# fan-ziqi/robot_lab

Hardware: AMD Instinct MI355X
Metric: env-steps/sec (whole node) at 4096 envs/GPU, A1 Velocity-Rough (higher is better)
Workload: dtype f32; 1 GPU; RobotLab-Isaac-Velocity-Rough-Unitree-A1-v0, 4096 envs/GPU, random actions U(-1,1), seed 42+rank; envs_per_gpu=4096, parallelism=env-shard x1, step_kernel=specialised (spec_id 1), envs_per_wavefront=4

## Files before the change

### robot_lab_amd/csrc/env_step.h

```cpp
#pragma once
#include <type_traits>

#include "env_spec.h"
#include "env_tables.h"

#if defined(RL_PHASE_MARKS) && defined(__HIP_DEVICE_COMPILE__)
#define RL_PHASE(id, name) asm volatile("; PHASE " name)
#elif defined(RL_PHASE_CLOCK) && defined(__HIP_DEVICE_COMPILE__)
#define RL_PHASE(id, name) this->phase_stamp(id)
#define RL_PHASE_START() (this->ph_t0 = 0, this->ph_cur = 0)
#define RL_PHASE_CLOCK_ON 1
#else
#define RL_PHASE(id, name) ((void)0)
#endif
#ifndef RL_PHASE_START
#define RL_PHASE_START() ((void)0)
#endif
constexpr int RL_PHASE_ROW0 = 24;
constexpr int RL_PHASE_SLOTS = 32;

namespace rl {

template <int N>
struct SymIdx {
  static constexpr int size = N * (N + 1) / 2;
  static constexpr int at(int i, int j) { return i <= j ? i * N - i * (i - 1) / 2 + (j - i) : j * N - j * (j - 1) / 2 + (i - j); }
};

template <int I, int N, class F>
RL_FN void static_for(F&& f) {
  if constexpr (I < N) {
    f(std::integral_constant<int, I>{});
    static_for<I + 1, N>(f);
  }
}
template <int I, class F>
RL_FN void static_for_down(F&& f) {
  if constexpr (I >= 0) {
    f(std::integral_constant<int, I>{});
    static_for_down<I - 1>(f);
  }
}

RL_FN float comp(V3 v, int i) { return i == 0 ? v.x : i == 1 ? v.y : v.z; }
RL_FN V3 unit(int i) { return {i == 0 ? 1.f : 0.f, i == 1 ? 1.f : 0.f, i == 2 ? 1.f : 0.f}; }
RL_FN V3 ld3(const float* p) { return {p[0], p[1], p[2]}; }

struct Uni {
  float dt, inv_dt, gravity, contact_k, contact_c, inv_phi_ref, contact_ct, contact_vdep, contact_vstick, limit_k, limit_c, force_threshold;
  float inv_hscale, x0, y0;
  int is_plane, nx, ny;
  double x0d, y0d, inv_hd;
  uint32_t trunk_restart;
};
template <class Ctx>
RL_FN Uni make_uni(const Ctx& ctx, const TaskTab& T) {
  Uni u;
  u.dt = ctx.uniform(T.dt); u.inv_dt = ctx.uniform(1.0f / T.dt); u.gravity = ctx.uniform(T.gravity);
  u.contact_k = ctx.uniform(T.contact_k); u.contact_c = ctx.uniform(T.contact_c); u.inv_phi_ref = ctx.uniform(1.0f / T.contact_phi_ref);
  u.contact_ct = ctx.uniform(T.contact_ct); u.contact_vdep = ctx.uniform(T.contact_vdep); u.contact_vstick = ctx.uniform(T.contact_vstick);
  u.limit_k = ctx.uniform(T.limit_k); u.limit_c = ctx.uniform(T.limit_c); u.force_threshold = ctx.uniform(T.force_threshold);
  u.inv_hscale = ctx.uniform(T.is_plane ? 1.0f : 1.0f / T.hscale); u.x0 = ctx.uniform(T.x0); u.y0 = ctx.uniform(T.y0);
  u.is_plane = ctx.uniform_i(T.is_plane); u.nx = ctx.uniform_i(T.nx); u.ny = ctx.uniform_i(T.ny);
  auto uni_d = [&](double v) {
    union { double d; int i[2]; } w;
    w.d = v;
    w.i[0] = ctx.uniform_i(w.i[0]); w.i[1] = ctx.uniform_i(w.i[1]);
    return w.d;
  };
// ... 490 lines not shown
    static_for<0, 3>([&](auto dc) __attribute__((always_inline)) {
      constexpr int D = 1 << decltype(dc)::value;
      float w[12] = {Rl.r0.x, Rl.r0.y, Rl.r0.z, Rl.r1.x, Rl.r1.y, Rl.r1.z, Rl.r2.x, Rl.r2.y, Rl.r2.z, pl.x, pl.y, pl.z};
      ctx.template sub_shr<D>(w);
      const M3 Rq{{w[0], w[1], w[2]}, {w[3], w[4], w[5]}, {w[6], w[7], w[8]}};
      const V3 pq{w[9], w[10], w[11]};
      const bool take = sub >= D;
      const M3 Rn = mul(Rq, Rl);
      const V3 pn = pq + mul(Rq, pl);
      Rl = select_m3(take, Rn, Rl);
      pl = select3(take, pn, pl);
    });
    const M3 Rj = mul(Ra, Rl);
    const V3 pj = pa + mul(Ra, pl);
    const V3 axj = mul(Rj, al_s);
    if (has) C.set(js, Rj, pj, axj);
    if constexpr (VEL) {
      const SV Sj{axj, cross(pj, axj)};
      const SV vj = Sj * (has ? qds : 0.f);
      float vs[6] = {vj.a.x, vj.a.y, vj.a.z, vj.l.x, vj.l.y, vj.l.z};
      static_for<0, 3>([&](auto dc) __attribute__((always_inline)) {
        constexpr int D = 1 << decltype(dc)::value;
        float w[6] = {vs[0], vs[1], vs[2], vs[3], vs[4], vs[5]};
        ctx.template sub_shr<D>(w);
        const bool take = sub >= D;
#pragma unroll
        for (int i = 0; i < 6; ++i) vs[i] += take ? w[i] : 0.f;
      });
      const SV Vj = Va + SV{{vs[0], vs[1], vs[2]}, {vs[3], vs[4], vs[5]}};
      const SV cj = crm(Vj, vj);
      float cs[6] = {cj.a.x, cj.a.y, cj.a.z, cj.l.x, cj.l.y, cj.l.z};
      static_for<0, 3>([&](auto dc) __attribute__((always_inline)) {
        constexpr int D = 1 << decltype(dc)::value;
        float w[6] = {cs[0], cs[1], cs[2], cs[3], cs[4], cs[5]};
        ctx.template sub_shr<D>(w);
        const bool take = sub >= D;
#pragma unroll
        for (int i = 0; i < 6; ++i) cs[i] += take ? w[i] : 0.f;
      });
      const SV aj = aa + SV{{cs[0], cs[1], cs[2]}, {cs[3], cs[4], cs[5]}};
      if (has) {
        float* w = va_words(js);
        st4(w, F4{Vj.a.x, Vj.a.y, Vj.a.z, Vj.l.x});
        st4(w + 4, F4{Vj.l.y, Vj.l.z, aj.a.x, aj.a.y});
        st4(w + 8, F4{aj.a.z, aj.l.x, aj.l.y, aj.l.z});
      }
    }
  }

  Ctx& ctx;
  const KState& S;
  const TablesT<TP>& T;
  const LaneTabT<TP>& L;
  const Uni u;
  int e, k, sub, li, Np;
  static constexpr int MAXOWN = SUB == 1 ? NBS : LaneTabT<TP>::template maxown<SUB>();
  int own[MAXOWN];
  static constexpr bool STATE_BUF = SUB == 1;
  float* lt;
  float* et;
  typename Ctx::StateBuf lt_b, et_b;
  uint32_t lt_off, et_off;
  struct BufRef {
    const typename Ctx::StateBuf& b;
    uint32_t voff, soff;
    RL_FN operator float() const { return Ctx::buf_ld(b, voff, soff); }
    RL_FN float operator=(float v) const { Ctx::buf_st(b, voff, soff, v); return v; }
  };
  struct PtrRef {
    float* p;
    RL_FN operator float() const { return *p; }
    RL_FN float operator=(float v) const { *p = v; return v; }
  };
  V3 pos, vlin, vang;
  Q4 quat;
  float q[JX], qd[JX], kp[JX], kd[JX], act[JX], prev_act[JX];
  V3 base_com;
  V3 wr_com;
  V3 extF, extT;
  float fric0[3];
  float tau_app[JX], qacc[JX];
  static constexpr int NOWN = LsFor<TP, Ctx::SUB>::NOWN;
  static constexpr bool GRAN = LsFor<TP, Ctx::SUB>::GRAN;
  LsMat<LSS, NOWN, 4, GRAN> tim;
  LsMat<LSS, NOWN, 3, GRAN> hist_n;
  LsMat<LSS, NOWN, 3, GRAN> cf;
  LsMat<LSS, NOWN, 3, GRAN> fric;

  RL_FN EnvLane(Ctx& c, const KState& s)
      : ctx(c), S(s), T(c.template tables<TablesT<TP>>()), L(c.template tables<TablesT<TP>>().lane[c.k()]), u(make_uni(c, c.template tables<TablesT<TP>>())), tim{c.template lane_scratch<GRAN>() + LS::TIM * LSS, {}}, hist_n{c.template lane_scratch<GRAN>() + LS::HIST * LSS, {}},
        cf{c.template lane_scratch<GRAN>() + LS::CF * LSS, {}}, fric{c.template lane_scratch<GRAN>() + LS::FRIC * LSS, {}} {
    e = ctx.env();
    k = ctx.k();
    sub = ctx.sub();
    li = k * SUB + sub;
    Np = S.Npad;
#pragma unroll
    for (int i = 0; i < MAXOWN; ++i) {
      if constexpr (SUB == 8) own[i] = -1;
      else own[i] = SUB == 1 ? i : (SUB == 2 ? L.own_slot2[sub & 1][i < LaneTabT<TP>::MAXOWN2 ? i : 0] : L.own_slot[sub & 3][i < LaneTabT<TP>::MAXOWN ? i : 0]);
    }
    if constexpr (SUB == 8) {
      int n = 0;
#pragma unroll
      for (int sl = 0; sl < NBS; ++sl) {
        const bool mine = (L.slot_body[sl] >= 0 || (sl == 0 && L.base_body_local >= 0)) && (L.slot_grp[sl] & 7) == sub;
#pragma unroll
        for (int i = 0; i < MAXOWN; ++i) own[i] = (mine && n == i) ? sl : own[i];
        n += mine ? 1 : 0;
      }
    }
    tim.set_own(own); hist_n.set_own(own); cf.set_own(own); fric.set_own(own);
    if constexpr (STATE_BUF) {
      lt_b = Ctx::state_buf(ctx.uniform_ptr(S.lane_state + (size_t)ctx.tile() * ((size_t)LY.NF_LANE * ROW)), (uint32_t)LY.NF_LANE * ROW * (uint32_t)sizeof(float));
      et_b = Ctx::state_buf(ctx.uniform_ptr(S.env_state + (size_t)ctx.tile() * ((size_t)LY.NF_ENV * EPT)), (uint32_t)LY.NF_ENV * (uint32_t)EPT * (uint32_t)sizeof(float));
      lt_off = (uint32_t)sizeof(float) * (uint32_t)(ctx.env_in_tile() * NLANE + k);
      et_off = (uint32_t)sizeof(float) * (uint32_t)ctx.env_in_tile();
    } else {
      lt = S.lane_state + (size_t)ctx.tile() * ((size_t)LY.NF_LANE * ROW) + (uint32_t)(ctx.env_in_tile() * NLANE + k);
      et = S.env_state + (size_t)ctx.tile() * ((size_t)LY.NF_ENV * EPT) + (uint32_t)ctx.env_in_tile();
    }
  }
#ifdef RL_PHASE_CLOCK_ON
  long long ph_t0 = 0;
  int ph_cur = 0;
  __device__ __forceinline__ void phase_stamp(int id) {
    __builtin_amdgcn_s_waitcnt(0);
    const long long t = (long long)__builtin_readcyclecounter();
    if (ctx.lane == 0 && ph_t0 != 0) {
      float* row = S.rew_terms + (size_t)RL_PHASE_ROW0 * (size_t)S.Npad + (size_t)ctx.tile() * RL_PHASE_SLOTS;
      row[ph_cur] += (float)(t - ph_t0);
    }
    ph_cur = id;
    __builtin_amdgcn_s_waitcnt(0);
    ph_t0 = (long long)__builtin_readcyclecounter();
  }
#endif
  RL_FN auto LF(int f) const {
    if constexpr (STATE_BUF) {
      const uint32_t o = (uint32_t)f * ROW * (uint32_t)sizeof(float);
      return __builtin_constant_p(f) ? BufRef{lt_b, lt_off, o} : BufRef{lt_b, lt_off + o, 0u};
    } else return PtrRef{lt + (uint32_t)f * ROW};
  }
  RL_FN auto EF(int f) const {
    if constexpr (STATE_BUF) {
      const uint32_t o = (uint32_t)f * (uint32_t)EPT * (uint32_t)sizeof(float);
      return __builtin_constant_p(f) ? BufRef{et_b, et_off, o} : BufRef{et_b, et_off + o, 0u};
    } else return PtrRef{et + (uint32_t)f * (uint32_t)EPT};
  }
  static constexpr bool M0 = TP::M0 != 0;
  static constexpr int G0 = M0 ? 1 : 0;
  RL_FN int grp_of(int it) const { return G0 + sub + SUB * it; }
  static constexpr bool slot_live(int it, int s) {
    const int lo = G0 + SUB * it, hi = lo + SUB - 1 < CL ? lo + SUB - 1 : CL;
    return spec_slot_any<SP>(s, SPL, lo, hi);
  }
  RL_FN bool owns_group(int g) const { return SUB == 1 || (g < G0 ? sub == 0 : ((g - G0) % SUB) == sub); }
  RL_FN bool on_base(int g, int s) const { return M0 && ((L.sph_base_mask >> (g * SPL + s)) & 1u) != 0u; }
  RL_FN static SV pick_sv(bool c, const SV& a, const SV& b) {
    return SV{{c ? a.a.x : b.a.x, c ? a.a.y : b.a.y, c ? a.a.z : b.a.z}, {c ? a.l.x : b.l.x, c ? a.l.y : b.l.y, c ? a.l.z : b.l.z}};
  }
  RL_FN uint32_t base_bits() const { return M0 ? L.sph_base_mask : ((1u << SPL) - 1u); }
  RL_FN bool owns_slot(int s) const { return owns_group(L.slot_grp[s]); }

  RL_FN void load() {
    pos = {EF(LY.EF_ROOT + 0), EF(LY.EF_ROOT + 1), EF(LY.EF_ROOT + 2)};
    quat = {EF(LY.EF_ROOT + 3), EF(LY.EF_ROOT + 4), EF(LY.EF_ROOT + 5), EF(LY.EF_ROOT + 6)};
    vlin = {EF(LY.EF_ROOT + 7), EF(LY.EF_ROOT + 8), EF(LY.EF_ROOT + 9)};
    vang = {EF(LY.EF_ROOT + 10), EF(LY.EF_ROOT + 11), EF(LY.EF_ROOT + 12)};
    extF = {EF(LY.EF_WRENCH + 0), EF(LY.EF_WRENCH + 1), EF(LY.EF_WRENCH + 2)};
    extT = {EF(LY.EF_WRENCH + 3), EF(LY.EF_WRENCH + 4), EF(LY.EF_WRENCH + 5)};
    base_com = {EF(LY.EF_BASE_COM + 0), EF(LY.EF_BASE_COM + 1), EF(LY.EF_BASE_COM + 2)};
    if (NW > 0) wr_com = {EF(LY.EF_WR_COM + 0), EF(LY.EF_WR_COM + 1), EF(LY.EF_WR_COM + 2)};
    else wr_com = base_com;
#pragma unroll
    for (int j = 0; j < CL; ++j) {
      q[j] = LF(LY.LF_Q + j);
      qd[j] = LF(LY.LF_QD + j);
      kp[j] = LF(LY.LF_KP + j);
      kd[j] = LF(LY.LF_KD + j);
      act[j] = LF(LY.LF_ACT + j);
    }
#pragma unroll
    for (int i = 0; i < NW; ++i) {
      q[CL + i] = EF(LY.EF_TQ + i);
      qd[CL + i] = EF(LY.EF_TQD + i);
      kp[CL + i] = EF(LY.EF_TKP + i);
      kd[CL + i] = EF(LY.EF_TKD + i);
      act[CL + i] = EF(LY.EF_TACT + i);
    }
#pragma unroll
    for (int j = 0; j < JX; ++j) {
      tau_app[j] = 0.f;
      qacc[j] = 0.f;
    }
    if (M0) {
#pragma unroll
      for (int t = 0; t < 3; ++t) fric0[t] = LF(LY.LF_FRICTION + t);
    }
#pragma unroll
    for (int i = 0; i < MAXOWN; ++i) {
      const int s = own[i];
      if (s < 0) continue;
      tim.st(s, F4{LF(LY.LF_TIMERS + s * 4 + 0), LF(LY.LF_TIMERS + s * 4 + 1), LF(LY.LF_TIMERS + s * 4 + 2), LF(LY.LF_TIMERS + s * 4 + 3)});
      fric.st(s, F4{LF(LY.LF_FRICTION + s * 3 + 0), LF(LY.LF_FRICTION + s * 3 + 1), LF(LY.LF_FRICTION + s * 3 + 2), 0.f});
      cf.st(s, F4{0.f, 0.f, 0.f, 0.f});
      hist_n.st(s, F4{0.f, 0.f, 0.f, 0.f});
    }
  }

  RL_FN void store() {
    if (li == 0) {
      EF(LY.EF_ROOT + 0) = pos.x; EF(LY.EF_ROOT + 1) = pos.y; EF(LY.EF_ROOT + 2) = pos.z;
      EF(LY.EF_ROOT + 3) = quat.w; EF(LY.EF_ROOT + 4) = quat.x; EF(LY.EF_ROOT + 5) = quat.y; EF(LY.EF_ROOT + 6) = quat.z;
      EF(LY.EF_ROOT + 7) = vlin.x; EF(LY.EF_ROOT + 8) = vlin.y; EF(LY.EF_ROOT + 9) = vlin.z;
      EF(LY.EF_ROOT + 10) = vang.x; EF(LY.EF_ROOT + 11) = vang.y; EF(LY.EF_ROOT + 12) = vang.z;
      EF(LY.EF_WRENCH + 0) = extF.x; EF(LY.EF_WRENCH + 1) = extF.y; EF(LY.EF_WRENCH + 2) = extF.z;
      EF(LY.EF_WRENCH + 3) = extT.x; EF(LY.EF_WRENCH + 4) = extT.y; EF(LY.EF_WRENCH + 5) = extT.z;
#pragma unroll
      for (int i = 0; i < NW; ++i) {
        EF(LY.EF_TQ + i) = q[CL + i];
        EF(LY.EF_TQD + i) = qd[CL + i];
        EF(LY.EF_TKP + i) = kp[CL + i];
        EF(LY.EF_TKD + i) = kd[CL + i];
        EF(LY.EF_TACT + i) = act[CL + i];
      }
    }
    if (sub == 0) {
#pragma unroll
      for (int j = 0; j < CL; ++j) {
        LF(LY.LF_Q + j) = q[j];
        LF(LY.LF_QD + j) = qd[j];
        LF(LY.LF_KP + j) = kp[j];
        LF(LY.LF_KD + j) = kd[j];
        LF(LY.LF_ACT + j) = act[j];
      }
    }
#pragma unroll
    for (int i = 0; i < MAXOWN; ++i) {
      const int s = own[i];
      if (s < 0 || (s == 0 && SUB > 1 && L.slot_body[0] < 0)) continue;
      const F4 t4 = tim.ld(s);
      LF(LY.LF_TIMERS + s * 4 + 0) = t4.x; LF(LY.LF_TIMERS + s * 4 + 1) = t4.y; LF(LY.LF_TIMERS + s * 4 + 2) = t4.z; LF(LY.LF_TIMERS + s * 4 + 3) = t4.w;
// ... 1170 lines not shown
```

### robot_lab_amd/csrc/env_terms.h

```cpp
#pragma once
#include "env_spec.h"
#include "env_step.h"

namespace rl {

enum RewKind {
  REW_TRACK_LIN_VEL_XY_EXP = 0, REW_TRACK_ANG_VEL_Z_EXP, REW_LIN_VEL_Z_L2, REW_ANG_VEL_XY_L2, REW_JOINT_TORQUES_L2,
  REW_JOINT_ACC_L2, REW_JOINT_POS_LIMITS, REW_JOINT_POWER, REW_STAND_STILL, REW_JOINT_POS_PENALTY, REW_JOINT_MIRROR,
  REW_ACTION_RATE_L2, REW_UNDESIRED_CONTACTS, REW_CONTACT_FORCES, REW_FEET_CONTACT_WITHOUT_CMD, REW_FEET_HEIGHT_BODY,
  REW_UPWARD, REW_FEET_AIR_TIME, REW_FEET_AIR_TIME_VARIANCE, REW_FEET_SLIDE, REW_FEET_GAIT, REW_FLAT_ORIENTATION_L2,
  REW_IS_TERMINATED, REW_JOINT_DEVIATION_L1, REW_JOINT_VEL_L2, REW_FEET_CONTACT, REW_FEET_STUMBLE, REW_FEET_HEIGHT,
  REW_TRACK_LIN_VEL_XY_YAW_FRAME_EXP, REW_TRACK_ANG_VEL_Z_WORLD_EXP, REW_FEET_AIR_TIME_POSITIVE_BIPED,
  REW_HANDSTAND_FEET_HEIGHT_EXP, REW_HANDSTAND_FEET_ON_AIR, REW_HANDSTAND_FEET_AIR_TIME, REW_HANDSTAND_ORIENTATION_L2, REW_BASE_HEIGHT_L2, REW_WHEEL_VEL_PENALTY,
  REW_FEET_DISTANCE_Y_EXP, REW_FEET_DISTANCE_XY_EXP, REW_ACTION_MIRROR, REW_ACTION_SYNC
};
enum ObsKind {
  OBS_BASE_LIN_VEL = 0, OBS_BASE_ANG_VEL, OBS_PROJECTED_GRAVITY, OBS_VELOCITY_COMMANDS, OBS_JOINT_POS_REL,
  OBS_JOINT_VEL_REL, OBS_LAST_ACTION, OBS_HEIGHT_SCAN, OBS_JOINT_POS_REL_NO_WHEEL
};

enum { JS_TAU2 = 0, JS_ACC2, JS_QD2, JS_LIMIT, JS_POWER, JS_DEV1, JS_DEV2, JS_DA2, JS_Q, JS_ABSQD, JS_ROWS };
enum { BT_HMAX = 0, BT_CA, BT_CC, BT_LA, BT_LC, BT_FX, BT_FY, BT_FZ, BT_PX, BT_PY, BT_PZ, BT_VX, BT_VY, BT_VZ, BT_NF };
static_assert(JS_ROWS == REW_JS_ROWS && BT_NF == REW_BT_NF && BT_FX == REW_BT_NS, "reward tables: LDS sizing in env_tables.h");

// ... 264 lines not shown
      }
      switch (R.kind) {
        case REW_UNDESIRED_CONTACTS: f = a0 * gate; break;
        case REW_CONTACT_FORCES: f = a0; break;
        case REW_FEET_CONTACT_WITHOUT_CMD: f = a0 * (cmd_norm < 0.1f ? 1.f : 0.f) * gate; break;
        case REW_FEET_CONTACT: f = (a0 != R.p[0] ? 1.f : 0.f) * moving * gate; break;
        case REW_FEET_AIR_TIME: f = a0 * moving * gate; break;
        case REW_HANDSTAND_FEET_AIR_TIME: f = a0; break;
        case REW_FEET_STUMBLE: f = (a0 > 0.f ? 1.f : 0.f) * gate; break;
        case REW_FEET_HEIGHT_BODY: case REW_FEET_HEIGHT: f = a0 * moving * gate; break;
        case REW_FEET_SLIDE: f = a0 * gate; break;
        case REW_FEET_AIR_TIME_POSITIVE_BIPED: f = (a0 == 1.f ? fminf(mn, R.p[0]) : 0.f) * moving * gate; break;
        case REW_HANDSTAND_FEET_HEIGHT_EXP: f = fexp(-a0 * frcp(R.p[0])); break;
        case REW_HANDSTAND_FEET_ON_AIR: f = a0 == 0.f ? 1.f : 0.f; break;
        case REW_FEET_AIR_TIME_VARIANCE: {
          const float inv_n = frcp(a0), inv_den = frcp(fmaxf(a0 - 1.f, 1.f));
          f = ((a2 - a1 * a1 * inv_n) + (a4 - a3 * a3 * inv_n)) * inv_den * gate;
        } break;
        default: break;
      }
    } break;
  }
  return f;
}


template <class Ctx, class TP, class SP = NoSpec>
struct EnvProgram : EnvLane<Ctx, TP, SP> {
  using Base = EnvLane<Ctx, TP, SP>;
  using ChainTP = typename Base::ChainTP;
  static constexpr Layout LY = Base::LY;
  static constexpr int CL = TP::CL, NW = TP::NW, JX = TP::JX, NBS = TP::NBS;
  using Base::ctx; using Base::S; using Base::T; using Base::L; using Base::e; using Base::k; using Base::sub; using Base::li; using Base::Np;
  static constexpr int SUB = Base::SUB;
  static constexpr int LPE = Base::LPE;
  using Base::pos; using Base::quat; using Base::vlin; using Base::vang; using Base::q; using Base::qd; using Base::kp; using Base::kd;
  using Base::act; using Base::prev_act; using Base::tim; using Base::cf; using Base::hist_n; using Base::tau_app; using Base::qacc;
  using Base::extF; using Base::extT; using Base::base_com; using Base::wr_com;

  V3 cmd;
  float heading_target, cmd_time_left, metric_xy, metric_yaw, push_left;
  static constexpr bool DEFER_LOG = SUB > 1;
  static constexpr int NACC_M = (MAX_T + LPE - 1) / LPE;
  float log_sum[NACC_M], log_mxy, log_myaw;
  bool is_heading, is_standing;
  int level, ttype;
  V3 origin;
  long long ep_len;
  M3 Rwb;
  V3 lin_b, ang_b, grav_b, lin_w;
  float yaw_c, yaw_s;

  RL_FN EnvProgram(Ctx& c, const KState& s) : Base(c, s) {}

  RL_FN void load_task() {
    cmd = {this->EF(LY.EF_CMD + CMD_VX), this->EF(LY.EF_CMD + CMD_VY), this->EF(LY.EF_CMD + CMD_WZ)};
    heading_target = this->EF(LY.EF_CMD + CMD_HEADING);
    cmd_time_left = this->EF(LY.EF_CMD + CMD_TIME_LEFT);
    metric_xy = this->EF(LY.EF_CMD + CMD_METRIC_XY);
    metric_yaw = this->EF(LY.EF_CMD + CMD_METRIC_YAW);
    push_left = this->EF(LY.EF_CMD + CMD_PUSH_LEFT);
    int f = S.flags[e];
    is_heading = f & 1;
    is_standing = (f >> 1) & 1;
    level = S.level[e];
    ttype = S.ttype[e];
    origin = {this->EF(LY.EF_ORIGIN + 0), this->EF(LY.EF_ORIGIN + 1), this->EF(LY.EF_ORIGIN + 2)};
    ep_len = S.ep_len[e];
  }
  RL_FN void store_task() {
    if (li != 0) return;
    this->EF(LY.EF_CMD + CMD_VX) = cmd.x; this->EF(LY.EF_CMD + CMD_VY) = cmd.y; this->EF(LY.EF_CMD + CMD_WZ) = cmd.z;
    this->EF(LY.EF_CMD + CMD_HEADING) = heading_target; this->EF(LY.EF_CMD + CMD_TIME_LEFT) = cmd_time_left;
    this->EF(LY.EF_CMD + CMD_METRIC_XY) = metric_xy; this->EF(LY.EF_CMD + CMD_METRIC_YAW) = metric_yaw; this->EF(LY.EF_CMD + CMD_PUSH_LEFT) = push_left;
    S.flags[e] = (is_heading ? 1 : 0) | (is_standing ? 2 : 0);
    S.level[e] = level;
    this->EF(LY.EF_ORIGIN + 0) = origin.x; this->EF(LY.EF_ORIGIN + 1) = origin.y; this->EF(LY.EF_ORIGIN + 2) = origin.z;
    S.ep_len[e] = ep_len;
    S.command_out[e * 3 + 0] = cmd.x; S.command_out[e * 3 + 1] = cmd.y; S.command_out[e * 3 + 2] = cmd.z;
  }

  RL_FN void derive() {
    Rwb = quat_to_mat(quat);
    V3 com_w = mul(Rwb, base_com);
    lin_w = vlin + cross(vang, com_w);
    lin_b = mulT(Rwb, lin_w);
    ang_b = mulT(Rwb, vang);
    grav_b = mulT(Rwb, V3{0.f, 0.f, -1.f});
    const float hn = frsqrt(fmaxf(Rwb.r0.x * Rwb.r0.x + Rwb.r1.x * Rwb.r1.x, 1e-30f));
    yaw_c = Rwb.r0.x * hn;
    yaw_s = Rwb.r1.x * hn;
  }

  RL_FN uint64_t uniform_u64(uint64_t v) const {
    return ((uint64_t)(uint32_t)ctx.uniform_i((int)(uint32_t)(v >> 32)) << 32) | (uint64_t)(uint32_t)ctx.uniform_i((int)(uint32_t)v);
  }
  RL_FN float U(uint32_t stream, uint32_t idx, float lo, float hi) const {
    return uniform_range(S.seed, (uint32_t)e, S.step_counter, stream, idx, lo, hi);
  }

  RL_FN void apply_command_draws(const float (&uw)[6]) {
    float rx0 = T.cmd_range[0][0], rx1 = T.cmd_range[0][1], ry0 = T.cmd_range[1][0], ry1 = T.cmd_range[1][1], rz0 = T.cmd_range[2][0], rz1 = T.cmd_range[2][1];
    float rh0 = T.cmd_range[3][0], rh1 = T.cmd_range[3][1], rel_h = T.cmd_rel_heading, rel_s = T.cmd_rel_standing, small = T.cmd_small_threshold;
    int use_heading = T.cmd_heading;
    rl_pin(rx0); rl_pin(rx1); rl_pin(ry0); rl_pin(ry1); rl_pin(rz0); rl_pin(rz1); rl_pin(rh0); rl_pin(rh1); rl_pin(rel_h); rl_pin(rel_s); rl_pin(small); rl_pin(use_heading);
    if (T.cur_lin != 0 || T.cur_ang != 0) {
// ... 841 lines not shown
        F[FEAT_JOINT + 2 * D + jid] = act[j];
        F[FEAT_JOINT + 3 * D + jid] = ((wheel >> (jid & 31)) & 1u) ? 0.f : qr;
      }
    }
    ctx.group_sync();
    const bool d0 = direct_group(T, 0), d1 = direct_group(T, 1);
    if (SUB == 1 && d0) write_group<true>(T.obs[0], F, S.obs_policy + (size_t)e * (size_t)T.policy_dim, 0u, cy, sy, scan_p, sp);
    else write_group<false>(T.obs[0], F, ctx.obs_stage(0), 0u, cy, sy, scan_p, sp);
    RL_PHASE(21, "obs.policy_done");
    if (SUB == 1 && d1) write_group<true>(T.obs[1], F, S.obs_critic + (size_t)e * (size_t)T.critic_dim, 1024u, cy, sy, scan_p, sp);
    else write_group<false>(T.obs[1], F, ctx.obs_stage(1), 1024u, cy, sy, scan_p, sp);
    RL_PHASE(22, "obs.flush");
    if (!(SUB == 1 && d0)) ctx.flush_obs(S.obs_policy, T.policy_dim, 0);
    if (!(SUB == 1 && d1)) ctx.flush_obs(S.obs_critic, T.critic_dim, 1);
  }

  RL_FN float* log_slot() const {
    return S.log + ((size_t)(S.step_counter & (uint32_t)(LOG_RING - 1)) * LOG_PARTS + (size_t)(ctx.tile() & (LOG_PARTS - 1))) * LOG_SIZE;
  }

  RL_FN void collect_cmd_levels(bool done) {
    if (!(T.cur_lin || T.cur_ang) || !done || e >= S.N || S.step_counter % (uint32_t)T.max_episode_length != 0u) return;
    for (int t = li; t < T.n_rewards; t += LPE) {
      const float v = S.ep_sums[(size_t)t * Np + e];
      if (T.cur_lin && t == T.cur_lin_term) { ctx.atomic_add(S.cmd_levels + CL_SUM_LIN, v); ctx.atomic_add(S.cmd_levels + CL_CNT_LIN, 1.f); }
      if (T.cur_ang && t == T.cur_ang_term) { ctx.atomic_add(S.cmd_levels + CL_SUM_ANG, v); ctx.atomic_add(S.cmd_levels + CL_CNT_ANG, 1.f); }
    }
  }
  RL_FN void write_dbg_views(float live) {
    if (S.dbg_torque == nullptr) return;
    if (sub == 0)
#pragma unroll
      for (int j = 0; j < JX; ++j) {
        if (TP::PAD && !L.joint_own[j]) continue;
        S.dbg_torque[(size_t)e * T.D + L.joint_id[j]] = live * tau_app[j];
        S.dbg_acc[(size_t)e * T.D + L.joint_id[j]] = live * qacc[j];
      }
#pragma unroll
    for (int s = 0; s < NBS; ++s) {
      int b = L.slot_body[s];
      if (b >= 0 && (s != 0 || L.owns_base_body) && this->owns_slot(s)) {
        float* o = S.dbg_cforce + ((size_t)e * T.n_bodies + b) * 3;
        const F4 fs = cf.ld(s);
        o[0] = live * fs.x; o[1] = live * fs.y; o[2] = live * fs.z;
      }
    }
  }
  RL_FN bool out_of_bounds() const {
    if (!T.term_oob || T.is_plane) return false;
    const float mw = (float)T.num_rows * T.tile_size + 2.f * T.border, mh = (float)T.num_cols * T.tile_size + 2.f * T.border;
    return fabsf(pos.x) > 0.5f * mw - T.oob_buffer || fabsf(pos.y) > 0.5f * mh - T.oob_buffer;
  }

  RL_FN void step() { step_front<false>(); }
  RL_FN void step_head() { step_front<true>(); }
  RL_FN void step_tail() {
    this->load();
    load_task();
    derive();
    const bool terminated = S.terminated[e] != 0, time_out = S.time_out[e] != 0;
    const bool t_oob = out_of_bounds();
    const bool t_timeout = T.term_time_out && ep_len >= (long long)T.max_episode_length;
    step_back<true>(terminated, time_out, t_timeout, t_oob, terminated);
  }

  template <bool HEAD>
  RL_FN void step_front() {
    constexpr size_t LOG_SLOT_WORDS = (size_t)LOG_PARTS * LOG_SIZE;
    const int log_tl = ctx.tile(), log_wl = ctx.env_in_tile() * LPE + li;
    float* log_pv = S.log + (size_t)((S.step_counter - 1u) & (uint32_t)(LOG_RING - 1)) * LOG_SLOT_WORDS;
    const float* log_pp = S.log + (size_t)((S.step_counter - 2u) & (uint32_t)(LOG_RING - 1)) * LOG_SLOT_WORDS;
    float log_fresh = 0.f, log_word = 0.f;
    if (log_tl < LOG_PARTS) {
      for (int p = 0; p < LOG_PARTS; ++p) log_fresh += log_pv[p * LOG_SIZE + LOG_FRESH];
      log_word = log_pp[log_tl * LOG_SIZE + log_wl];
    }
    float a_in[JX];
    {
      const float* arow = S.action_in + (size_t)(e < S.N ? e : 0) * T.D;
#pragma unroll
      for (int j = 0; j < JX; ++j) {
        const int jid = L.joint_id[j];
        a_in[j] = arow[TP::PAD && jid < 0 ? 0 : jid];
      }
    }
    RL_PHASE_START();
    RL_PHASE(0, "load");
    this->load();
    load_task();
    rl_pin(a_in);
    if (log_tl < LOG_PARTS) {
      float* nx = S.log + (size_t)((S.step_counter + 1u) & (uint32_t)(LOG_RING - 1)) * LOG_SLOT_WORDS;
      const bool inherit = log_fresh == 0.f;
      if (inherit && log_wl != LOG_FRESH) log_pv[log_tl * LOG_SIZE + log_wl] = log_word;
      nx[log_tl * LOG_SIZE + log_wl] = 0.f;
      for (int p = log_tl + S.Npad / (64 / LPE); p < LOG_PARTS; p += S.Npad / (64 / LPE)) {
        if (inherit && log_wl != LOG_FRESH) log_pv[p * LOG_SIZE + log_wl] = log_pp[p * LOG_SIZE + log_wl];
        nx[p * LOG_SIZE + log_wl] = 0.f;
      }
    }
    RL_PHASE(1, "action");
    float q_tgt[JX], qd_tgt[JX];
#pragma unroll
    for (int j = 0; j < JX; ++j) {
      prev_act[j] = act[j];
      const float a = (e < S.N && (!TP::PAD || L.joint_id[j] >= 0)) ? a_in[j] : 0.f;
      act[j] = a;
      float pr = clampf(a * L.a_scale[j] + L.a_off[j], L.a_lo[j], L.a_hi[j]);
      q_tgt[j] = L.action_is_vel[j] ? 0.f : pr;
      qd_tgt[j] = L.action_is_vel[j] ? pr : 0.f;
    }
#ifdef RL_ABL_SUBSTEPS
    if constexpr (Base::ABA) {
      this->substeps_aba(q_tgt, qd_tgt, RL_ABL_SUBSTEPS);
    } else
#endif
    if constexpr (Base::ABA) {
      this->substeps_aba(q_tgt, qd_tgt, T.decimation);
    } else {
      this->self_load();
      for (int s = 0; s < T.decimation; ++s) this->substep_aba_trunk(q_tgt, qd_tgt);
    }
    RL_PHASE(15, "terminations");
    ep_len += 1;
    derive();
    if constexpr (NW > 0) {
      ChainTP Cf = this->new_chain();
      this->kinematics(Cf);
      ctx.group_sync();
    }

    bool t_timeout = T.term_time_out && ep_len >= (long long)T.max_episode_length;
    const bool t_oob = out_of_bounds();
    bool t_illegal = false;
    if (T.term_illegal) {
      const uint64_t ill_mask = T.illegal_body_mask;
      const float ill_thr = T.illegal_threshold;
      float c = 0.f;
#pragma unroll
      for (int i = 0; i < Base::MAXOWN; ++i) {
        const int so = this->own[i], s = so < 0 ? 0 : so;
        const float h = hist_max(s);
// ... 137 lines not shown
```

### robot_lab_amd/csrc/rl_env_kernels.h

```cpp
#pragma once
#include <hip/hip_runtime.h>

#include <algorithm>
#include <cmath>
#include <cstdlib>
#include <mutex>
#include <string>

#define RL_FN __host__ __device__ __forceinline__
#include "env_aos.h"
#include "env_terms.h"

namespace {

using namespace rl;

template <int CTRL>
__device__ inline float dpp(float v) {
  return __int_as_float(__builtin_amdgcn_update_dpp(0, __float_as_int(v), CTRL, 0xF, 0xF, false));
}
template <int CTRL>
__device__ inline float dpp_move(float v) {
  return __int_as_float(__builtin_amdgcn_update_dpp(0, __float_as_int(v), CTRL, 0xF, 0xF, true));
}
// ... 173 lines not shown
  }
};

struct LdsPlan {
  int s0w, s1w;
  int fdim, rtdim, rsdim;
  int lb0, lbrec0, envs, tail;
  int rstage, stage0, stage1, fstage;
  int words;
};
template <class TP, int SUB>
RL_FN LdsPlan lds_plan(int policy_dim, int critic_dim, bool direct0, bool direct1, int D, int n_bodies, uint64_t rew_ext_mask, int n_rewards) {
  constexpr int EPT = 64 / (NLANE * SUB), LIMBS = 64 / SUB;
  using LS = typename LsFor<TP, SUB>::type;
  constexpr int STASH_WORDS = LsFor<TP, SUB>::STASH * LsFor<TP, SUB>::type::SSW * 64;
  constexpr int LB_FREE = TP::NW > 0 ? LbLayout<TP>::RECW * LIMBS : 0;
  LdsPlan P;
  P.s0w = (SUB == 1 && direct0) ? 0 : (EPT * policy_dim + 3) & ~3;
  P.s1w = (SUB == 1 && direct1) ? 0 : (EPT * critic_dim + 3) & ~3;
  P.fdim = feat_count(D);
  P.rtdim = rew_tab_words(D, n_bodies, rew_ext_mask);
  P.rsdim = rew_stage_words(n_rewards);
  int region = P.s0w + P.s1w + EPT * P.fdim;
  if (region < EPT * P.rtdim) P.s1w += EPT * P.rtdim - region, region = EPT * P.rtdim;
  if (SUB > 1 && region < EPT * RESET_RAND_WORDS) P.s1w += EPT * RESET_RAND_WORDS - region, region = EPT * RESET_RAND_WORDS;
  P.lb0 = LS::WORDS * 64;
  P.lbrec0 = P.lb0 + LbLayout<TP>::CHAINW * LIMBS;
  P.envs = P.lb0 + LbLayout<TP>::WORDS * LIMBS;
  P.tail = P.envs + EPT * LbLayout<TP>::ENV_WORDS;
  const bool alias = TP::NW == 0 && STASH_WORDS > 0 && EPT * P.rsdim + region <= STASH_WORDS;
  const bool alias_lb = TP::NW > 0 && EPT * P.rsdim + region <= LB_FREE;
  P.rstage = alias ? LS::CT * 64 : (alias_lb ? P.lbrec0 : P.tail);
  P.stage0 = P.rstage + EPT * P.rsdim;
  P.stage1 = P.stage0 + P.s0w;
  P.fstage = P.stage1 + P.s1w;
  P.words = (alias || alias_lb) ? P.tail : P.tail + EPT * P.rsdim + region;
  P.words = (P.words + 3) & ~3;
  return P;
}

extern __shared__ float4 smem4[];

#ifndef RL_LB
#define RL_LB(w) 256
#endif
template <class TP, int RESET, int SUB, int WGW, class SP = NoSpec>
__global__ __launch_bounds__(RL_LB(WGW)) void env_kernel(KState S, const void* __restrict__ Tgv, uint32_t wave_words) {
  using Ctx = WaveCtx<SUB>;
  using Tables = TablesT<TP>;
  const Tables* __restrict__ Tg = static_cast<const Tables*>(Tgv);
  float* smem = reinterpret_cast<float*>(smem4);
  Tables* Tl = reinterpret_cast<Tables*>(smem);
  const int lane = threadIdx.x & 63, wv = threadIdx.x >> 6;
  S.step_counter += *S.step_base;
  {
    const float4* src = reinterpret_cast<const float4*>(Tg);
    float4* dst = reinterpret_cast<float4*>(Tl);
    constexpr int TPB = 64 * WGW;
    constexpr int NIT = ((int)(sizeof(Tables) / 16) + TPB - 1) / TPB;
    const int n4 = (int)(S.table_bytes >> 4);
    float4 tmp[NIT];
#pragma unroll
    for (int it = 0; it < NIT; ++it) {
      const int i = (int)threadIdx.x + TPB * it;
      tmp[it] = src[i < n4 ? i : n4 - 1];
    }
#pragma unroll
    for (int it = 0; it < NIT; ++it) {
      const int i = (int)threadIdx.x + TPB * it;
      if (i < n4) dst[i] = tmp[it];
    }
  }
  if (WGW > 1) __syncthreads();
  else Ctx::wave_sync();
  const int TAB_F = (int)(S.table_bytes >> 2);
  const LdsPlan P = lds_plan<TP, SUB>(Tl->policy_dim, Tl->critic_dim, direct_group(*Tl, 0), direct_group(*Tl, 1), Tl->D, Tl->n_bodies, Tl->rew_ext_mask, Tl->n_rewards);
  Ctx ctx;
  ctx.T = Tl;
  ctx.Tg = Tgv;
  ctx.dim[0] = Tl->policy_dim;
  ctx.dim[1] = Tl->critic_dim;
  ctx.lscratch = smem + TAB_F + (WGW > 1 ? wv * wave_words : 0u);
  ctx.wtile = (int)blockIdx.x * WGW + wv;
  if (WGW > 1 && ctx.wtile >= S.Npad / Ctx::EPT) return;
  ctx.lbchain = ctx.lscratch + P.lb0 + (lane / SUB) * LbLayout<TP>::CHAINW;
  ctx.lbrec = ctx.lscratch + P.lbrec0 + (lane / SUB) * LbLayout<TP>::RECW;
  ctx.lbrec_stride = LbLayout<TP>::RECW;
  ctx.envs = ctx.lscratch + P.envs + (lane / Ctx::LPE) * LbLayout<TP>::ENV_WORDS;
  ctx.fdim = P.fdim;
  ctx.rtdim = P.rtdim;
  ctx.rsdim = P.rsdim;
  ctx.rstage = ctx.lscratch + P.rstage;
  ctx.stage[0] = ctx.lscratch + P.stage0;
  ctx.stage[1] = ctx.lscratch + P.stage1;
  ctx.fstage = ctx.lscratch + P.fstage;
  ctx.lane = lane;
  EnvProgram<Ctx, TP, SP> prog(ctx, S);
  if (RESET == 1)
    prog.reset_entry();
  else if (RESET == 2)
    prog.step_head();
  else
    prog.step();
}


struct LaunchCfg {
  int device = 0, n_cu = 256;
  int wg_waves = 4;
  bool wg_force = false;
};

template <class TP, int SUB, int WGW, class SP = NoSpec>
hipError_t launch_w(const LaunchCfg& cfg, const KState& S, const void* T, size_t lds1, hipStream_t st) {
  const int tiles = S.Npad / (16 / SUB);
  dim3 grid((tiles + WGW - 1) / WGW), block(64 * WGW);
  const uint32_t wave_words = (uint32_t)((lds1 - S.table_bytes) >> 2);
  const size_t lds = S.table_bytes + (size_t)WGW * (lds1 - S.table_bytes);
  constexpr bool HEAD = SUB == 4 && WGW == 1 && !SP::ON, RESET = WGW == 1 && !SP::ON;
  if (lds > 64 * 1024) {
    static size_t configured[64] = {};
    static std::mutex mu;
    std::lock_guard<std::mutex> lock(mu);
    size_t& have = configured[cfg.device & 63];
    if (lds > have) {
      hipError_t e = hipFuncSetAttribute(reinterpret_cast<const void*>(&env_kernel<TP, 0, SUB, WGW, SP>), hipFuncAttributeMaxDynamicSharedMemorySize, (int)lds);
      if (e != hipSuccess) return e;
      if constexpr (RESET) {
        e = hipFuncSetAttribute(reinterpret_cast<const void*>(&env_kernel<TP, 1, SUB, WGW>), hipFuncAttributeMaxDynamicSharedMemorySize, (int)lds);
        if (e != hipSuccess) return e;
      }
      if constexpr (HEAD) {
        e = hipFuncSetAttribute(reinterpret_cast<const void*>(&env_kernel<TP, 2, SUB, WGW>), hipFuncAttributeMaxDynamicSharedMemorySize, (int)lds);
        if (e != hipSuccess) return e;
      }
      have = lds;
    }
  }
  if (S.mode == KMODE_RESET || S.mode == KMODE_STEP_TAIL) {
    if constexpr (RESET) hipLaunchKernelGGL((env_kernel<TP, 1, SUB, WGW>), grid, block, lds, st, S, T, wave_words);
    else return hipErrorInvalidValue;
  } else if (S.mode == KMODE_STEP_HEAD) {
    if constexpr (HEAD) hipLaunchKernelGGL((env_kernel<TP, 2, SUB, WGW>), grid, block, lds, st, S, T, wave_words);
    else return hipErrorInvalidValue;
  } else {
    hipLaunchKernelGGL((env_kernel<TP, 0, SUB, WGW, SP>), grid, block, lds, st, S, T, wave_words);
  }
  return hipGetLastError();
}
inline bool four_wave_workgroup(const LaunchCfg& cfg, int NW, int sub, int tiles, size_t lds1, size_t table_bytes) {
  return (NW == 0 || sub == 8) && cfg.wg_waves == 4 && (tiles >= 4 * cfg.n_cu || cfg.wg_force) && table_bytes + 4 * (lds1 - table_bytes) <= 160 * 1024;
}
template <class TP, int SUB, class SP = NoSpec>
hipError_t launch_cl(const LaunchCfg& cfg, const KState& S, const void* T, size_t lds1, hipStream_t st) {
  if constexpr (TP::NW == 0 || SUB == 8) {
    if (four_wave_workgroup(cfg, TP::NW, SUB, S.Npad / (16 / SUB), lds1, S.table_bytes) && S.mode == KMODE_STEP)
// ... 42 lines not shown
```

### robot_lab_amd/csrc/rl_math.h

```cpp
#pragma once
#include <math.h>
#include <stdint.h>

#ifndef RL_FN
#define RL_FN inline
#endif

namespace rl {

#if defined(__HIP_DEVICE_COMPILE__)
RL_FN void rl_pin(float& x) { asm volatile("" : "+v"(x)); }
RL_FN void rl_pin(int& x) { asm volatile("" : "+v"(x)); }
#else
RL_FN void rl_pin(float&) {}
RL_FN void rl_pin(int&) {}
#endif
template <int N>
RL_FN void rl_pin(float (&a)[N]) {
#pragma unroll
  for (int i = 0; i < N; ++i) rl_pin(a[i]);
}

#if defined(__HIP_DEVICE_COMPILE__) && !defined(RL_EXACT_MATH)
RL_FN float frcp(float x) { return __builtin_amdgcn_rcpf(x); }
RL_FN float fsqrt(float x) { return __builtin_amdgcn_sqrtf(x); }
RL_FN float frsqrt(float x) { return __builtin_amdgcn_rsqf(x); }
#else
RL_FN float frcp(float x) { return 1.0f / x; }
RL_FN float fsqrt(float x) { return sqrtf(x); }
RL_FN float frsqrt(float x) { return 1.0f / sqrtf(x); }
#endif
RL_FN float fdiv(float a, float b) { return a * frcp(b); }
#if defined(__HIP_DEVICE_COMPILE__) && !defined(RL_EXACT_MATH)
RL_FN float fexp(float x) { return __builtin_amdgcn_exp2f(x * 1.44269504088896340736f); }
#else
RL_FN float fexp(float x) { return expf(x); }
#endif
#if defined(__HIP_DEVICE_COMPILE__)
RL_FN float opaque(float x) {
  asm("" : "+v"(x));
  return x;
}
#else
RL_FN float opaque(float x) { return x; }
#endif
#if defined(__HIP_DEVICE_COMPILE__)
typedef float F2p __attribute__((ext_vector_type(2)));
RL_FN F2p pk_fma(F2p a, F2p b, F2p c) { return __builtin_elementwise_fma(a, b, c); }
#else
struct F2p {
  float x, y;
};
RL_FN F2p pk_fma(F2p a, F2p b, F2p c) { return F2p{fmaf(a.x, b.x, c.x), fmaf(a.y, b.y, c.y)}; }
#endif
#if defined(__HIP_DEVICE_COMPILE__)
RL_FN F2p pk_mul(F2p a, F2p b) { return a * b; }
RL_FN F2p pk_add(F2p a, F2p b) { return a + b; }
#else
RL_FN F2p pk_mul(F2p a, F2p b) { return F2p{a.x * b.x, a.y * b.y}; }
RL_FN F2p pk_add(F2p a, F2p b) { return F2p{a.x + b.x, a.y + b.y}; }
#endif
RL_FN F2p pk2(float a, float b) { return F2p{a, b}; }
RL_FN F2p pk1(float a) { return F2p{a, a}; }

RL_FN float ftanh(float x) {
  return 1.0f - 2.0f * frcp(fexp(2.0f * fminf(x, 20.0f)) + 1.0f);
}

// ... 165 lines not shown
```

Baseline: 131.4 million env-steps/s.

## Issue env state loads early to overlap with table copy into LDS

Constructs the env program before the table-to-LDS copy and issues the per-env state, joint and task loads while the table global loads are still in flight, so their latencies overlap instead of running back to back. A compile-time budget picks how many loads to hoist based on the register count. The workgroup barrier becomes a hand-written s_barrier with a narrower waitcnt, and out-of-range waves are clamped rather than returning before the barrier. This raises register pressure during the prologue and depends on the fence and waitcnt encoding being correct.

```diff
diff --git a/robot_lab_amd/csrc/env_step.h b/robot_lab_amd/csrc/env_step.h
--- a/robot_lab_amd/csrc/env_step.h
+++ b/robot_lab_amd/csrc/env_step.h
@@ -4,17 +4,23 @@
 #include "env_spec.h"
 #include "env_tables.h"
 
+constexpr int RL_PHASE_ID_START = 25;
 #if defined(RL_PHASE_MARKS) && defined(__HIP_DEVICE_COMPILE__)
 #define RL_PHASE(id, name) asm volatile("; PHASE " name)
+#define RL_PHASE_ENTRY() asm volatile("; PHASE start")
 #elif defined(RL_PHASE_CLOCK) && defined(__HIP_DEVICE_COMPILE__)
 #define RL_PHASE(id, name) this->phase_stamp(id)
-#define RL_PHASE_START() (this->ph_t0 = 0, this->ph_cur = 0)
+#define RL_PHASE_ENTRY() const long long rl_phase_entry = (long long)__builtin_readcyclecounter()
+#define RL_PHASE_START(prog) ((prog).ph_t0 = rl_phase_entry, (prog).ph_cur = RL_PHASE_ID_START)
 #define RL_PHASE_CLOCK_ON 1
 #else
 #define RL_PHASE(id, name) ((void)0)
 #endif
 #ifndef RL_PHASE_START
-#define RL_PHASE_START() ((void)0)
+#define RL_PHASE_START(prog) ((void)0)
+#endif
+#ifndef RL_PHASE_ENTRY
+#define RL_PHASE_ENTRY() ((void)0)
 #endif
 constexpr int RL_PHASE_ROW0 = 24;
 constexpr int RL_PHASE_SLOTS = 32;
@@ -611,7 +617,7 @@
   const KState& S;
   const TablesT<TP>& T;
   const LaneTabT<TP>& L;
-  const Uni u;
+  Uni u;
   int e, k, sub, li, Np;
   static constexpr int MAXOWN = SUB == 1 ? NBS : LaneTabT<TP>::template maxown<SUB>();
   int own[MAXOWN];
@@ -646,30 +652,16 @@
   LsMat<LSS, NOWN, 3, GRAN> cf;
   LsMat<LSS, NOWN, 3, GRAN> fric;
 
-  RL_FN EnvLane(Ctx& c, const KState& s)
-      : ctx(c), S(s), T(c.template tables<TablesT<TP>>()), L(c.template tables<TablesT<TP>>().lane[c.k()]), u(make_uni(c, c.template tables<TablesT<TP>>())), tim{c.template lane_scratch<GRAN>() + LS::TIM * LSS, {}}, hist_n{c.template lane_scratch<GRAN>() + LS::HIST * LSS, {}},
+  struct Deferred {};
+  RL_FN EnvLane(Ctx& c, const KState& s) : EnvLane(c, s, Deferred{}) { setup(); }
+  RL_FN EnvLane(Ctx& c, const KState& s, Deferred)
+      : ctx(c), S(s), T(c.template tables<TablesT<TP>>()), L(c.template tables<TablesT<TP>>().lane[c.k()]), tim{c.template lane_scratch<GRAN>() + LS::TIM * LSS, {}}, hist_n{c.template lane_scratch<GRAN>() + LS::HIST * LSS, {}},
         cf{c.template lane_scratch<GRAN>() + LS::CF * LSS, {}}, fric{c.template lane_scratch<GRAN>() + LS::FRIC * LSS, {}} {
     e = ctx.env();
     k = ctx.k();
     sub = ctx.sub();
     li = k * SUB + sub;
     Np = S.Npad;
-#pragma unroll
-    for (int i = 0; i < MAXOWN; ++i) {
-      if constexpr (SUB == 8) own[i] = -1;
-      else own[i] = SUB == 1 ? i : (SUB == 2 ? L.own_slot2[sub & 1][i < LaneTabT<TP>::MAXOWN2 ? i : 0] : L.own_slot[sub & 3][i < LaneTabT<TP>::MAXOWN ? i : 0]);
-    }
-    if constexpr (SUB == 8) {
-      int n = 0;
-#pragma unroll
-      for (int sl = 0; sl < NBS; ++sl) {
-        const bool mine = (L.slot_body[sl] >= 0 || (sl == 0 && L.base_body_local >= 0)) && (L.slot_grp[sl] & 7) == sub;
-#pragma unroll
-        for (int i = 0; i < MAXOWN; ++i) own[i] = (mine && n == i) ? sl : own[i];
-        n += mine ? 1 : 0;
-      }
-    }
-    tim.set_own(own); hist_n.set_own(own); cf.set_own(own); fric.set_own(own);
     if constexpr (STATE_BUF) {
       lt_b = Ctx::state_buf(ctx.uniform_ptr(S.lane_state + (size_t)ctx.tile() * ((size_t)LY.NF_LANE * ROW)), (uint32_t)LY.NF_LANE * ROW * (uint32_t)sizeof(float));
       et_b = Ctx::state_buf(ctx.uniform_ptr(S.env_state + (size_t)ctx.tile() * ((size_t)LY.NF_ENV * EPT)), (uint32_t)LY.NF_ENV * (uint32_t)EPT * (uint32_t)sizeof(float));
@@ -679,6 +671,25 @@
       lt = S.lane_state + (size_t)ctx.tile() * ((size_t)LY.NF_LANE * ROW) + (uint32_t)(ctx.env_in_tile() * NLANE + k);
       et = S.env_state + (size_t)ctx.tile() * ((size_t)LY.NF_ENV * EPT) + (uint32_t)ctx.env_in_tile();
     }
+  }
+  RL_FN void setup() {
+    u = make_uni(ctx, T);
+#pragma unroll
+    for (int i = 0; i < MAXOWN; ++i) {
+      if constexpr (SUB == 8) own[i] = -1;
+      else own[i] = SUB == 1 ? i : (SUB == 2 ? L.own_slot2[sub & 1][i < LaneTabT<TP>::MAXOWN2 ? i : 0] : L.own_slot[sub & 3][i < LaneTabT<TP>::MAXOWN ? i : 0]);
+    }
+    if constexpr (SUB == 8) {
+      int n = 0;
+#pragma unroll
+      for (int sl = 0; sl < NBS; ++sl) {
+        const bool mine = (L.slot_body[sl] >= 0 || (sl == 0 && L.base_body_local >= 0)) && (L.slot_grp[sl] & 7) == sub;
+#pragma unroll
+        for (int i = 0; i < MAXOWN; ++i) own[i] = (mine && n == i) ? sl : own[i];
+        n += mine ? 1 : 0;
+      }
+    }
+    tim.set_own(own); hist_n.set_own(own); cf.set_own(own); fric.set_own(own);
   }
 #ifdef RL_PHASE_CLOCK_ON
   long long ph_t0 = 0;
@@ -722,7 +733,13 @@
   RL_FN uint32_t base_bits() const { return M0 ? L.sph_base_mask : ((1u << SPL) - 1u); }
   RL_FN bool owns_slot(int s) const { return owns_group(L.slot_grp[s]); }
 
+  static constexpr int EARLY_STATE_LOADS = 13 + 6 + 3 + (NW > 0 ? 3 : 0), EARLY_JOINT_LOADS = 5 * CL + 5 * NW;
   RL_FN void load() {
+    load_early<true>();
+    load_late<2>();
+  }
+  template <bool JOINTS>
+  RL_FN void load_early() {
     pos = {EF(LY.EF_ROOT + 0), EF(LY.EF_ROOT + 1), EF(LY.EF_ROOT + 2)};
     quat = {EF(LY.EF_ROOT + 3), EF(LY.EF_ROOT + 4), EF(LY.EF_ROOT + 5), EF(LY.EF_ROOT + 6)};
     vlin = {EF(LY.EF_ROOT + 7), EF(LY.EF_ROOT + 8), EF(LY.EF_ROOT + 9)};
@@ -732,6 +749,9 @@
     base_com = {EF(LY.EF_BASE_COM + 0), EF(LY.EF_BASE_COM + 1), EF(LY.EF_BASE_COM + 2)};
     if (NW > 0) wr_com = {EF(LY.EF_WR_COM + 0), EF(LY.EF_WR_COM + 1), EF(LY.EF_WR_COM + 2)};
     else wr_com = base_com;
+    if constexpr (JOINTS) load_joints();
+  }
+  RL_FN void load_joints() {
 #pragma unroll
     for (int j = 0; j < CL; ++j) {
       q[j] = LF(LY.LF_Q + j);
@@ -748,6 +768,10 @@
       kd[CL + i] = EF(LY.EF_TKD + i);
       act[CL + i] = EF(LY.EF_TACT + i);
     }
+  }
+  template <int EARLY>
+  RL_FN void load_late() {
+    if constexpr (EARLY < 2) load_joints();
 #pragma unroll
     for (int j = 0; j < JX; ++j) {
       tau_app[j] = 0.f;
diff --git a/robot_lab_amd/csrc/env_terms.h b/robot_lab_amd/csrc/env_terms.h
--- a/robot_lab_amd/csrc/env_terms.h
+++ b/robot_lab_amd/csrc/env_terms.h
@@ -340,6 +340,10 @@
   float yaw_c, yaw_s;
 
   RL_FN EnvProgram(Ctx& c, const KState& s) : Base(c, s) {}
+  using Deferred = typename Base::Deferred;
+  RL_FN EnvProgram(Ctx& c, const KState& s, Deferred d) : Base(c, s, d) {}
+  static constexpr int EARLY_ENV_LOADS = Base::EARLY_STATE_LOADS + 15;
+  static constexpr int EARLY_JOINT_LOADS = Base::EARLY_JOINT_LOADS;
 
   RL_FN void load_task() {
     cmd = {this->EF(LY.EF_CMD + CMD_VX), this->EF(LY.EF_CMD + CMD_VY), this->EF(LY.EF_CMD + CMD_WZ)};
@@ -1287,8 +1291,9 @@
     return fabsf(pos.x) > 0.5f * mw - T.oob_buffer || fabsf(pos.y) > 0.5f * mh - T.oob_buffer;
   }
 
-  RL_FN void step() { step_front<false>(); }
-  RL_FN void step_head() { step_front<true>(); }
+  template <int EARLY = 0>
+  RL_FN void step() { step_front<false, EARLY>(); }
+  RL_FN void step_head() { step_front<true, 0>(); }
   RL_FN void step_tail() {
     this->load();
     load_task();
@@ -1299,10 +1304,10 @@
     step_back<true>(terminated, time_out, t_timeout, t_oob, terminated);
   }
 
-  template <bool HEAD>
+  template <bool HEAD, int EARLY>
   RL_FN void step_front() {
     constexpr size_t LOG_SLOT_WORDS = (size_t)LOG_PARTS * LOG_SIZE;
-    const int log_tl = ctx.tile(), log_wl = ctx.env_in_tile() * LPE + li;
+    const int log_tl = ctx.uniform_i(ctx.tile()), log_wl = ctx.env_in_tile() * LPE + li;
     float* log_pv = S.log + (size_t)((S.step_counter - 1u) & (uint32_t)(LOG_RING - 1)) * LOG_SLOT_WORDS;
     const float* log_pp = S.log + (size_t)((S.step_counter - 2u) & (uint32_t)(LOG_RING - 1)) * LOG_SLOT_WORDS;
     float log_fresh = 0.f, log_word = 0.f;
@@ -1319,10 +1324,12 @@
         a_in[j] = arow[TP::PAD && jid < 0 ? 0 : jid];
       }
     }
-    RL_PHASE_START();
     RL_PHASE(0, "load");
-    this->load();
-    load_task();
+    if constexpr (EARLY > 0) this->template load_late<EARLY>();
+    else {
+      this->load();
+      load_task();
+    }
     rl_pin(a_in);
     if (log_tl < LOG_PARTS) {
       float* nx = S.log + (size_t)((S.step_counter + 1u) & (uint32_t)(LOG_RING - 1)) * LOG_SLOT_WORDS;
diff --git a/robot_lab_amd/csrc/rl_env_kernels.h b/robot_lab_amd/csrc/rl_env_kernels.h
--- a/robot_lab_amd/csrc/rl_env_kernels.h
+++ b/robot_lab_amd/csrc/rl_env_kernels.h
@@ -249,12 +249,24 @@
   float* smem = reinterpret_cast<float*>(smem4);
   Tables* Tl = reinterpret_cast<Tables*>(smem);
   const int lane = threadIdx.x & 63, wv = threadIdx.x >> 6;
-  S.step_counter += *S.step_base;
+  constexpr int TPB = 64 * WGW;
+  constexpr int NIT = ((int)(sizeof(Tables) / 16) + TPB - 1) / TPB;
+  using Prog = EnvProgram<Ctx, TP, SP>;
+  constexpr int EARLY = RESET != 0 ? 0 : (NIT + Prog::EARLY_ENV_LOADS + Prog::EARLY_JOINT_LOADS <= 60 ? 2 : (NIT + Prog::EARLY_ENV_LOADS <= 60 ? 1 : 0));
+  uint32_t step_base = *S.step_base;
+  RL_PHASE_ENTRY();
+  const int TAB_F = (int)(S.table_bytes >> 2);
+  const int wtile = (int)blockIdx.x * WGW + wv, ntile = S.Npad / Ctx::EPT;
+  Ctx ctx;
+  ctx.T = Tl;
+  ctx.Tg = Tgv;
+  ctx.lscratch = smem + TAB_F + (WGW > 1 ? wv * wave_words : 0u);
+  ctx.wtile = (WGW > 1 && wtile >= ntile) ? ntile - 1 : wtile;
+  ctx.lane = lane;
+  Prog prog(ctx, S, typename Prog::Deferred{});
   {
     const float4* src = reinterpret_cast<const float4*>(Tg);
     float4* dst = reinterpret_cast<float4*>(Tl);
-    constexpr int TPB = 64 * WGW;
-    constexpr int NIT = ((int)(sizeof(Tables) / 16) + TPB - 1) / TPB;
     const int n4 = (int)(S.table_bytes >> 4);
     float4 tmp[NIT];
 #pragma unroll
@@ -262,24 +274,36 @@
       const int i = (int)threadIdx.x + TPB * it;
       tmp[it] = src[i < n4 ? i : n4 - 1];
     }
+    if constexpr (EARLY > 0) {
+      __builtin_amdgcn_sched_barrier(0);
+      prog.template load_early<EARLY == 2>();
+      prog.load_task();
+      rl_pin_uniform(step_base);
+    }
+    if constexpr (RESET == 0) {
+#pragma unroll
+      for (int it = 0; it < NIT; ++it) { rl_pin(tmp[it].x); rl_pin(tmp[it].y); rl_pin(tmp[it].z); rl_pin(tmp[it].w); }
+    }
 #pragma unroll
     for (int it = 0; it < NIT; ++it) {
       const int i = (int)threadIdx.x + TPB * it;
-      if (i < n4) dst[i] = tmp[it];
-    }
-  }
-  if (WGW > 1) __syncthreads();
-  else Ctx::wave_sync();
-  const int TAB_F = (int)(S.table_bytes >> 2);
+      if constexpr (RESET == 0) dst[i < n4 ? i : n4 - 1] = tmp[it];
+      else if (i < n4) dst[i] = tmp[it];
+    }
+  }
+  if (WGW > 1) {
+    if constexpr (EARLY > 0) {
+      __builtin_amdgcn_fence(__ATOMIC_ACQ_REL, "wavefront");
+      __builtin_amdgcn_s_waitcnt(0xC07F);
+      __builtin_amdgcn_s_barrier();
+      __builtin_amdgcn_fence(__ATOMIC_ACQ_REL, "wavefront");
+    } else __syncthreads();
+  } else Ctx::wave_sync();
+  if (WGW > 1 && wtile >= ntile) return;
+  S.step_counter += step_base;
   const LdsPlan P = lds_plan<TP, SUB>(Tl->policy_dim, Tl->critic_dim, direct_group(*Tl, 0), direct_group(*Tl, 1), Tl->D, Tl->n_bodies, Tl->rew_ext_mask, Tl->n_rewards);
-  Ctx ctx;
-  ctx.T = Tl;
-  ctx.Tg = Tgv;
   ctx.dim[0] = Tl->policy_dim;
   ctx.dim[1] = Tl->critic_dim;
-  ctx.lscratch = smem + TAB_F + (WGW > 1 ? wv * wave_words : 0u);
-  ctx.wtile = (int)blockIdx.x * WGW + wv;
-  if (WGW > 1 && ctx.wtile >= S.Npad / Ctx::EPT) return;
   ctx.lbchain = ctx.lscratch + P.lb0 + (lane / SUB) * LbLayout<TP>::CHAINW;
   ctx.lbrec = ctx.lscratch + P.lbrec0 + (lane / SUB) * LbLayout<TP>::RECW;
   ctx.lbrec_stride = LbLayout<TP>::RECW;
@@ -291,14 +315,15 @@
   ctx.stage[0] = ctx.lscratch + P.stage0;
   ctx.stage[1] = ctx.lscratch + P.stage1;
   ctx.fstage = ctx.lscratch + P.fstage;
-  ctx.lane = lane;
-  EnvProgram<Ctx, TP, SP> prog(ctx, S);
+  prog.setup();
   if (RESET == 1)
     prog.reset_entry();
   else if (RESET == 2)
     prog.step_head();
-  else
-    prog.step();
+  else {
+    RL_PHASE_START(prog);
+    prog.template step<EARLY>();
+  }
 }
 
 
diff --git a/robot_lab_amd/csrc/rl_math.h b/robot_lab_amd/csrc/rl_math.h
--- a/robot_lab_amd/csrc/rl_math.h
+++ b/robot_lab_amd/csrc/rl_math.h
@@ -11,9 +11,11 @@
 #if defined(__HIP_DEVICE_COMPILE__)
 RL_FN void rl_pin(float& x) { asm volatile("" : "+v"(x)); }
 RL_FN void rl_pin(int& x) { asm volatile("" : "+v"(x)); }
+RL_FN void rl_pin_uniform(uint32_t& x) { asm volatile("" : "+s"(x)); }
 #else
 RL_FN void rl_pin(float&) {}
 RL_FN void rl_pin(int&) {}
+RL_FN void rl_pin_uniform(uint32_t&) {}
 #endif
 template <int N>
 RL_FN void rl_pin(float (&a)[N]) {
```

New measurement: 132.8 million env-steps/s (median of 6 runs). 1.1% higher.
